# SteveMacenski/slam_toolbox

Measured on AMD Instinct MI355X. Metric: scan-matches/sec, higher is better.
Workload: dtype u8 gather / i32 sum / f64 penalty; 1 GPU; BASELINE config[1]: CorrelateScan 1081 beams 61x61x81 poses; parallelism=1 x independent match shards (no collective), streams_per_gpu=1

## Files before the change

### include/karto_hip.h

```cpp
#ifndef KARTO_HIP_H_
#define KARTO_HIP_H_

#include <stdint.h>

#ifdef __cplusplus
extern "C" {
#endif

#define KH_API __attribute__((visibility("default")))

enum {
  KH_OK = 0,
  KH_ERR_INVALID_ARG = 1,
  KH_ERR_NO_DEVICE = 2,
  KH_ERR_HIP = 3,
  KH_ERR_SEARCH = 4,
  KH_ERR_NOT_FOUND = 5,
  KH_ERR_SOLVER = 6,
  KH_ERR_IO = 7
};

KH_API const char * kh_last_error(void);
KH_API int kh_device_count(void);
KH_API const char * kh_version(void);
// ... 84 lines not shown
                                         double best_response, const double center[3], double angle_offset,
                                         double angle_resolution, double cov[9]);

typedef struct kh_grid_info {
  int32_t width, height, width_step, data_size;
  int32_t roi_x, roi_y, roi_w, roi_h;
  int32_t kernel_size;
  int32_t search_side;
  double offset_x, offset_y, scale;
} kh_grid_info;
KH_API int kh_matcher_grid_info(kh_matcher * m, int32_t slot, kh_grid_info * out);
KH_API int kh_matcher_read_grid(kh_matcher * m, int32_t slot, uint8_t * out );
KH_API int kh_matcher_read_kernel(kh_matcher * m, uint8_t * out );
KH_API int kh_matcher_read_lookup(kh_matcher * m, int32_t slot, int32_t * n_angles,
                                  int32_t * n_points, int32_t * out);
KH_API int kh_matcher_read_volume(kh_matcher * m, int32_t slot, int32_t * nx, int32_t * ny,
                                  int32_t * na, int32_t * out_sums, double * out_responses);
KH_API int kh_matcher_read_search_probabilities(kh_matcher * m, int32_t slot, int32_t * nx, int32_t * ny, double * out);
KH_API int kh_matcher_set_debug(kh_matcher * m, int32_t flags);
KH_API int kh_matcher_seq_stats(kh_matcher * m, int64_t out[8]);
KH_API void * kh_matcher_stream(kh_matcher * m);
KH_API int kh_matcher_profile(kh_matcher * m, int32_t enable, double * score_ms, int64_t * score_launches,
                              double * raster_ms, int64_t * raster_launches);

KH_API int kh_matcher_profile_side(kh_matcher * m, double * offsets_ms, double * ties_ms);

KH_API int kh_matcher_score_loads(kh_matcher * m, int64_t * wave_loads, int32_t reset);

typedef struct kh_spa kh_spa;

// ... 472 lines not shown
```

### slam_toolbox_amd/capi.py

```python
from __future__ import annotations

import ctypes as C
import os

import numpy as np

HERE = os.path.dirname(os.path.abspath(__file__))
LIB_PATH = os.environ.get("KH_LIBRARY") or os.path.join(HERE, "libkartohip.so")

KH_OK, KH_ERR_INVALID_ARG, KH_ERR_NO_DEVICE, KH_ERR_HIP, KH_ERR_SEARCH, KH_ERR_NOT_FOUND, KH_ERR_SOLVER, KH_ERR_IO = range(8)
KH_GRAPH_TEXT, KH_GRAPH_BINARY = 0, 1

dptr = np.ctypeslib.ndpointer(dtype=np.float64, flags="C_CONTIGUOUS")
iptr = np.ctypeslib.ndpointer(dtype=np.int32, flags="C_CONTIGUOUS")
bptr = np.ctypeslib.ndpointer(dtype=np.uint8, flags="C_CONTIGUOUS")


class KhScan(C.Structure):
    _fields_ = [("n", C.c_int32), ("ranges", C.POINTER(C.c_double)), ("points_xy", C.POINTER(C.c_double)),
                ("sensor_pose", C.c_double * 3), ("device_points_xy", C.c_void_p)]


class KhMatchParams(C.Structure):
    _fields_ = [("coarse_search_angle_offset", C.c_double), ("coarse_angle_resolution", C.c_double),
# ... 69 lines not shown
KH_SPA_MAX_COV_COLUMNS = 64


class KhMarginalizeSummary(C.Structure):
    _fields_ = [(k, C.c_int32) for k in ("n_marginalized", "n_plain", "n_rounds", "n_added", "n_fused", "max_degree")] + \
               [(k, C.c_double) for k in ("pack_ms", "kernel_ms", "apply_ms", "total_ms")]


KH_REMOVE_PLAIN, KH_REMOVE_MARGINALIZE = 0, 1


SYMBOLS = [
    "kh_last_error", "kh_device_count", "kh_version", "kh_scan_points", "kh_match_params_default",
    "kh_matcher_create", "kh_matcher_destroy", "kh_matcher_set_params", "kh_matcher_match",
    "kh_matcher_match_batch", "kh_matcher_add_scans", "kh_matcher_correlate", "kh_matcher_correlate_batch",
    "kh_matcher_grid_info", "kh_matcher_read_grid", "kh_matcher_read_kernel", "kh_matcher_read_lookup",
    "kh_matcher_positional_covariance", "kh_matcher_angular_covariance",
    "kh_matcher_read_volume", "kh_matcher_read_search_probabilities", "kh_matcher_set_debug", "kh_matcher_stream", "kh_matcher_profile", "kh_matcher_score_loads", "kh_matcher_seq_stats", "kh_matcher_profile_side",
    "kh_matcher_group_create", "kh_matcher_group_destroy", "kh_matcher_group_set_params", "kh_matcher_group_size", "kh_matcher_group_member",
    "kh_matcher_group_device", "kh_matcher_group_match_batch", "kh_loop_closure_batch",
    "kh_spa_options_default", "kh_spa_create", "kh_spa_set_debug", "kh_spa_destroy", "kh_spa_set_options", "kh_spa_reset",
    "kh_spa_clear", "kh_spa_add_node", "kh_spa_add_constraint", "kh_spa_remove_node",
    "kh_spa_remove_constraint", "kh_spa_modify_node", "kh_spa_get_node", "kh_spa_num_nodes",
    "kh_spa_num_constraints", "kh_spa_compute", "kh_spa_iteration_log", "kh_spa_get_corrections", "kh_link_info", "kh_spa_set_sharding",
    "kh_spa_save", "kh_spa_load", "kh_spa_add_constraint_information", "kh_spa_get_node_at", "kh_spa_get_constraint", "kh_spa_get_nodes",
    "kh_graph_create", "kh_graph_destroy", "kh_graph_set", "kh_graph_set_positions", "kh_graph_find_loop_candidates",
    "kh_graph_last_kernel_ms", "kh_graph_find_near_chains", "kh_graph_closest_scan_to_pose", "kh_weighted_mean",
    "kh_occupancy_compute_dimensions", "kh_occupancy_create", "kh_occupancy_destroy", "kh_occupancy_clear",
    "kh_occupancy_add_scans", "kh_occupancy_update", "kh_occupancy_read", "kh_occupancy_info",
    "kh_decay_params_default", "kh_lifelong_scores", "kh_lifelong_scores_resident",
    "kh_spa_set_comm", "kh_comm_unique_id", "kh_comm_create", "kh_comm_destroy", "kh_comm_rank", "kh_comm_world", "kh_comm_device",
# ... 187 lines not shown
        L.kh_matcher_group_member.argtypes = [vp, i32]
        L.kh_matcher_group_member.restype = vp
        L.kh_matcher_group_device.argtypes = [vp, i32]
        L.kh_matcher_group_match_batch.argtypes = [vp, i32, C.POINTER(KhScan), C.POINTER(KhScan), iptr, vp, i32, i32, dptr, dptr, dptr, iptr]
        L.kh_loop_closure_batch.argtypes = [vp, vp, i32, C.POINTER(KhScan), C.POINTER(KhScan), iptr, dbl, dbl, dbl, dbl, i32,
                                            dptr, dptr, dptr, iptr, dptr, dptr, dptr]
    L.kh_matcher_add_scans.argtypes = [vp, i32, C.POINTER(KhScan), C.POINTER(KhScan), i32]
    L.kh_matcher_correlate.argtypes = [vp, i32, C.POINTER(KhScan), dptr, dptr, dptr, dbl, dbl, i32, i32, dptr, dptr, C.POINTER(dbl)]
    L.kh_matcher_correlate_batch.argtypes = [vp, i32, C.POINTER(KhScan), dptr, dptr, dptr, dbl, dbl, i32, i32, dptr, dptr, dptr, iptr]
    L.kh_matcher_positional_covariance.argtypes = [vp, i32, dptr, dbl, dptr, dptr, dptr, dbl, dptr]
    L.kh_matcher_angular_covariance.argtypes = [vp, i32, C.POINTER(KhScan), dptr, dbl, dptr, dbl, dbl, dptr]
    L.kh_matcher_grid_info.argtypes = [vp, i32, C.POINTER(KhGridInfo)]
    L.kh_matcher_read_grid.argtypes = [vp, i32, bptr]
    L.kh_matcher_read_kernel.argtypes = [vp, bptr]
    L.kh_matcher_read_lookup.argtypes = [vp, i32, C.POINTER(i32), C.POINTER(i32), vp]
    L.kh_matcher_read_volume.argtypes = [vp, i32, C.POINTER(i32), C.POINTER(i32), C.POINTER(i32), vp, vp]
    if hasattr(L, "kh_matcher_read_search_probabilities"):
        L.kh_matcher_read_search_probabilities.argtypes = [vp, i32, C.POINTER(i32), C.POINTER(i32), vp]
    L.kh_matcher_set_debug.argtypes = [vp, i32]
    L.kh_matcher_stream.argtypes = [vp]
    L.kh_matcher_stream.restype = vp
    L.kh_matcher_profile.argtypes = [vp, i32, C.POINTER(dbl), C.POINTER(C.c_int64), C.POINTER(dbl), C.POINTER(C.c_int64)]
    L.kh_matcher_score_loads.argtypes = [vp, C.POINTER(C.c_int64), i32]
    L.kh_matcher_seq_stats.argtypes = [vp, C.POINTER(C.c_int64)]
    L.kh_matcher_profile_side.argtypes = [vp, C.POINTER(C.c_double), C.POINTER(C.c_double)]
    if hasattr(L, "kh_spa_create"):
        L.kh_spa_options_default.argtypes = [C.POINTER(KhSpaOptions)]
        L.kh_spa_create.argtypes = [i32, C.POINTER(vp)]
        L.kh_spa_destroy.argtypes = [vp]
        L.kh_spa_destroy.restype = None
# ... 219 lines not shown
```

### slam_toolbox_amd/csrc/kh_internal.hpp

```cpp
#pragma once
#include <cstddef>
#include <cstdint>

namespace kh
{

constexpr int32_t kInvalidScan = INT32_MAX;
constexpr int32_t kOccupied = 100;
constexpr int32_t kTieCap = 2048;
constexpr int32_t kGridPad = 512;
constexpr int32_t kTileBytes = 64;
constexpr int32_t kTileSpan = 61;
constexpr int32_t kClasses = 4;
constexpr int32_t kBlockShift = 5;
constexpr int32_t kCountsPerAngle = 8;
#ifndef KH_GROUP_ANGLES
#define KH_GROUP_ANGLES 2
#endif
#ifndef KH_LDS_PITCH
#define KH_LDS_PITCH 192
#endif
#ifndef KH_LDS_ROWS
#define KH_LDS_ROWS 196
#endif
// ... 94 lines not shown
  int32_t bm_w, bm_h, bshift;
  double * tile_best;
  int32_t * sums;
  double * resp;
  unsigned long long * out;
  int32_t out_words;
  const uint8_t * grid2;
  int32_t pitch2, copy_b;
  int32_t * fast2;
  int32_t * tcounts2;
  int32_t dec;
  int32_t pad_rows;
  int32_t pad;
  int32_t tile_px;
  unsigned long long * load_counter;
};

constexpr size_t kOutHeaderWords = 2 + kTieCap / 2;

struct ValidItem {int32_t job, scan;};
void launch_find_valid(const RasterJob * d_jobs, const ValidItem * d_items, int32_t n_items, int32_t max_n, void * stream);
void launch_active_set(const RasterJob * d_jobs, int32_t n_jobs, int32_t max_points, int32_t max_cap, void * stream);
void launch_raster(const RasterJob * d_jobs, int32_t n_jobs, int32_t max_points, int32_t max_tiles, const uint8_t * d_kernel, int32_t kernel_size,
  void * stream);
void launch_raster_clear(const RasterJob * d_jobs, int32_t n_jobs, void * stream);
void launch_repitch(const RasterJob * d_jobs, int32_t n_jobs, int32_t max_tiles, void * stream, bool any_copies);
void launch_repitch_full(const RasterJob * d_job, int32_t rows, void * stream);
void launch_offsets(const uint8_t * d_jobs, size_t stride, int32_t n_jobs, int32_t max_na, void * stream);
void launch_score(const uint8_t * d_jobs, size_t stride, int32_t n_jobs, int32_t max_tiles, int32_t max_na,
                  int32_t sx_variant, int32_t ry, void * stream);
__host__ __device__ inline int32_t lds_row_waves(int32_t ny) {return ny <= 16 ? 1 : ny <= 32 ? 2 : 4;}
inline int32_t score_tile_poses(int32_t sx) {return sx == 2 ? (kTileSpan + 1) / 2 : kTileSpan;}
void launch_offsets_lds(const uint8_t * d_jobs, size_t stride, int32_t n_jobs, int32_t max_na, void * stream);
void launch_score_lds(const uint8_t * d_jobs, size_t stride, int32_t n_jobs, int32_t max_na, int32_t sx_variant, bool full_rows, void * stream);
void launch_gather_small(const uint8_t * d_jobs, size_t stride, int32_t n_jobs, int32_t * d_out, int32_t small_stride, void * stream);
void launch_ties(const uint8_t * d_jobs, size_t stride, int32_t n_jobs, int32_t max_poses, int32_t tile_pairs, bool cells_in_score, void * stream);

}
```

### slam_toolbox_amd/csrc/matcher_device.hpp

```cpp
#pragma once
#include <hip/hip_runtime.h>
#include <atomic>
#include <cstdint>
#include "kh_internal.hpp"
#include "lds_attr.hpp"

namespace kh
{

__device__ __forceinline__ double d_round(double v) {return v >= 0.0 ? floor(v + 0.5) : ceil(v - 0.5);}
__device__ __forceinline__ int32_t d_to_int(double v)
{
  if (!(v > -2147483649.0 && v < 2147483648.0)) {return INT32_MIN;}
  return (int32_t)v;
}
__device__ __forceinline__ double2 job_point(const RasterJob & job, int p)
{
  if (job.uniform_n > 0) {
    const int k = p / job.uniform_n;
    return reinterpret_cast<const double2 *>(job.scan_ptr[k])[p - k * job.uniform_n];
  }
  int lo = 0, hi = job.n_scans;
  while (hi - lo > 1) {
    const int mid = (lo + hi) >> 1;
// ... 36 lines not shown
  const unsigned long long span = (1ull << nb) - 1ull;
  typedef __attribute__((address_space(1))) const uint32_t gword;
  gword * const words = (gword *)bmp + wi;
  constexpr int kRowsAtOnce = 9;
  unsigned long long any = 0;
  for (int by = by0; by <= by1; by += kRowsAtOnce) {
    uint32_t lo[kRowsAtOnce], hi[kRowsAtOnce];
#pragma unroll
    for (int k = 0; k < kRowsAtOnce; ++k) {
      gword * row = words + (size_t)min(by + k, by1) * bm_w;
      lo[k] = row[0]; hi[k] = row[1];
    }
#pragma unroll
    for (int k = 0; k < kRowsAtOnce; ++k) {any |= ((unsigned long long)hi[k] << 32) | lo[k];}
  }
  return ((any >> sh) & span) != 0;
}

template <bool kWaveSearch>
__device__ __forceinline__ void find_valid_scan(const double2 * pts, const int n, uint8_t * out, const double vx, const double vy,
  const int max_n, double2 * s_fv, uint8_t *& flags_lds, long long * dbg = nullptr)
{
#define KH_FV_STAMP(k) do {if (dbg && threadIdx.x == 0) {dbg[k] = (long long)wall_clock64();}} while (0)
  const int tid = threadIdx.x, lane = tid & 63, nthreads = blockDim.x;
  const int stride_i = max_n + 64;
  double2 * P = s_fv;
  int32_t * nxt0 = reinterpret_cast<int32_t *>(P + max_n);
  int32_t * nxa = nxt0 + stride_i;
  int32_t * nxb = nxa + stride_i;
  uint8_t * reach = reinterpret_cast<uint8_t *>(nxb + stride_i);
// ... 225 lines not shown
```

### slam_toolbox_amd/csrc/matcher_host.cpp

```cpp
#include "matcher_private.hpp"
#include "matcher_seq.hpp"

namespace kh
{
thread_local std::string g_last_error;
void set_error(const std::string & s) {g_last_error = s;}
}


namespace kh
{

static int32_t half_kernel_size(double smear, double resolution)
{
  return static_cast<int32_t>(round_half_away(2.0 * smear / resolution));
}


void host_parallel_for(size_t n, const std::function<void(size_t)> & fn) {HostPool::instance().run(n, fn);}
void host_parallel_for_wide(size_t n, const std::function<void(size_t)> & fn) {HostPool::wide().run(n, fn);}

void fill_raster_job(const kh_matcher * m, const Slot & s, const double * pose, int32_t n_points, size_t npad, RasterJob & j)
{
  std::memset(&j, 0, sizeof(j));
  j.grid = s.d_grid;
  j.view_x = pose[0]; j.view_y = pose[1];
  j.active = s.d_ractive; j.n_points = n_points;
  j.ws = m->ws; j.roi_x = m->roi_x; j.roi_y = m->roi_y; j.roi_w = m->roi_w; j.roi_h = m->roi_h;
  j.kernel_size = m->kernel_size; j.off_x = s.off_x; j.off_y = s.off_y; j.scale = m->scale;
  j.blockmap = s.d_blockmap; j.bm_w = m->bm_w; j.bm_h = m->bm_h; j.bshift = m->bshift;
  const size_t nt = static_cast<size_t>(m->rt_w) * m->rt_h;
  j.tiles_w = m->rt_w; j.tiles_h = m->rt_h; j.height = m->data_size / m->ws;
  j.tile_count = s.d_rtiles; j.tile_cursor = s.d_rtiles + nt; j.n_work = s.d_rtiles + 2 * nt;
  j.tile_start = s.d_rtiles + 2 * nt + 4; j.work = s.d_rtiles + 3 * nt + 4;
  j.cell_xy = s.d_rlists; j.list = s.d_rlists + 2 * npad; j.rank = s.d_rlists + 6 * npad;
  j.grid2 = s.d_grid2; j.copy_kind = s.copy_kind; j.prev_work = s.d_prev_work;
  j.pitch2 = s.copy_kind == 2 ? m->pitch_d : m->pitch2; j.copy_b = s.copy_kind == 2 ? m->copy_q : m->copy_b;
  j.n_foot = static_cast<int32_t>(m->footprint100.size()) - 1;
// ... 519 lines not shown
  job->grid_off_x = s.off_x; job->grid_off_y = s.off_y; job->scale = m->scale;
  job->bx = reinterpret_cast<const int32_t *>(db + L.bx);
  job->by = reinterpret_cast<const int32_t *>(db + L.by);
  job->dist_pen = L.dist_pen_bytes ? reinterpret_cast<const double *>(db + L.dist_pen) : c.geo->d_dist_pen;
  job->ang_pen = reinterpret_cast<const double *>(db + L.ang_pen);
  job->cos_sin = reinterpret_cast<const double *>(db + L.cos_sin);
  job->local = reinterpret_cast<const double *>(db + L.local);
  job->invalid = db + L.invalid;
  job->table = s.d_table; job->fast = s.d_fast; job->slow = s.d_slow; job->counts = s.d_counts;
  job->tcounts = s.d_tcounts; {
    const int32_t tiles = job->tiles_x * job->tiles_y;
    job->list_tiles = (tiles >= 4 && tiles <= c.lt_alloc) ? tiles : 1;
  }
  job->sums = s.d_sums; job->resp = s.d_resp; job->out = d_out; job->out_words = static_cast<int32_t>(out_words);
  job->blockmap = m->dense_score ? nullptr : s.d_blockmap; job->bm_w = m->bm_w; job->bm_h = m->bm_h; job->bshift = m->bshift;
  job->tile_best = s.d_tile_best;
  {
    const bool use2 = dec || (s.copy_kind == 1 && m->dual_copy && linear && (job->tiles_x == 1 || job->list_tiles > 1));
    const size_t lists = static_cast<size_t>(c.na) * kClasses * static_cast<size_t>(c.lt_alloc);
    job->grid2 = use2 ? s.d_grid2 : nullptr;
    job->pitch2 = dec ? m->pitch_d : m->pitch2; job->copy_b = dec ? m->copy_q : m->copy_b;
    job->fast2 = s.d_fast + lists * static_cast<size_t>(c.P);
    job->tcounts2 = s.d_tcounts + lists;
  }
  job->pad = std::max(0, m->pad_rows * m->ws - 512); job->pad_rows = m->pad_rows;
  job->load_counter = m->profiling ? m->d_load_counter : nullptr;
}

int finalize_job(kh_matcher * m, CorrReq & q, CorrHost & c, const ResultView & v)
{
// ... 171 lines not shown
    std::fprintf(stderr, "[kh corr] job 0: %d x %d x %d poses, sx %d, tiles %d x %d of %d x %d poses, lists per tile %d, copies %d (slot kind %d), "
      "dec %d, ws %d\n", j0->nx, j0->ny, j0->na, j0->sx, j0->tiles_x, j0->tiles_y, j0->tile_px, 4 * j0->ry, j0->list_tiles,
      j0->grid2 ? 1 : 0, m->slots[B.ctx[0].slot].copy_kind, j0->dec, m->ws);
  }
  int32_t max_tiles = 0, sx_variant = shapes[0].sx, ry = shapes[0].ry;
  const int32_t lds_sx = shapes[0].lds_sx;
  bool uniform_kernel = true, all_lds = true;
  for (size_t i = 0; i < n; ++i) {
    if (sx_variant != shapes[i].sx || ry != shapes[i].ry) {uniform_kernel = false;}
    all_lds = all_lds && shapes[i].lds_sx == lds_sx;
    max_tiles = std::max(max_tiles, shapes[i].tiles);
    all_lds = all_lds && shapes[i].lds != 0;
  }
  B.use_lds = all_lds && uniform_kernel;
  int32_t tile_pairs = 0;
  for (size_t i = 0; i < n; ++i) {
    CorrJob * job = reinterpret_cast<CorrJob *>(B.h_stage + stride * i);
    if (B.use_lds) {
      job->tiles_x = 1; job->tiles_y = 1; job->ry = 16; job->tile_px = kTileSpan;
      job->cells_in_score = 1;
    }
    tile_pairs = std::max(tile_pairs, job->na * job->tiles_x * job->tiles_y);
  }

  timing.lap(0, t_enter);
  const auto t_enqueue = std::chrono::steady_clock::now();
  hipStream_t cs = overlap ? B.side : m->stream;
  KH_HIP(hipMemcpyAsync(B.d_stage, B.h_stage, stride * n, hipMemcpyHostToDevice, cs));
  if (m->profiling) {KH_HIP(hipEventRecord(B.evs[0], cs));}
  if (B.use_lds) {
    launch_offsets_lds(B.d_stage, stride, static_cast<int32_t>(n), max_na, cs);
  } else {
    launch_offsets(B.d_stage, stride, static_cast<int32_t>(n), max_na, cs);
  }
  if (m->profiling) {KH_HIP(hipEventRecord(B.evs[1], cs));}
  if (m->profiling) {KH_HIP(hipEventRecord(B.ev[0], cs));}
  if (B.use_lds) {
    bool full_rows = true;
    for (size_t i = 0; i < n; ++i) {full_rows = full_rows && lds_row_waves(B.ctx[i].ny) == 4;}
    launch_score_lds(B.d_stage, stride, static_cast<int32_t>(n), max_na, lds_sx, full_rows, cs);
  } else if (uniform_kernel) {
    launch_score(B.d_stage, stride, static_cast<int32_t>(n), max_tiles, max_na, sx_variant, ry, cs);
  } else {
    for (size_t i = 0; i < n; ++i) {
      const CorrJob * job = reinterpret_cast<const CorrJob *>(B.h_stage + stride * i);
// ... 281 lines not shown
  }
  m->rt_w = (m->ws + kRasterTile - 1) / kRasterTile;
  m->rt_h = (m->data_size / m->ws + kRasterTile - 1) / kRasterTile;
  m->bshift = (m->kernel_size <= 25 && m->side <= 64 && max_batch >= 8) ? 3 : kBlockShift;
  m->bm_w = (((m->ws >> m->bshift) + 1) + 31) / 32 + 1;
  m->bm_h = (m->data_size / m->ws >> m->bshift) + 2;
  {
    const double table_bytes = 4.0 * static_cast<double>(m->roi_w) * m->roi_h * max_batch;
    m->table_raster = table_bytes <= 24e9 && m->rt_w * m->rt_h <= 16384;
  }
  m->slots.resize(max_batch);
  for (auto & s : m->slots) {
    if ((e = hipMalloc(reinterpret_cast<void **>(&s.d_grid_alloc), static_cast<size_t>(m->data_size) + 2 * m->grid_pad)) != hipSuccess) {return fail(e, "hipMalloc grid");}
    if ((e = hipMemset(s.d_grid_alloc, 0, static_cast<size_t>(m->data_size) + 2 * m->grid_pad)) != hipSuccess) {return fail(e, "hipMemset grid");}
    s.d_grid = s.d_grid_alloc + m->grid_pad;
    if ((e = hipMalloc(reinterpret_cast<void **>(&s.d_blockmap), static_cast<size_t>(m->bm_w) * m->bm_h * 4)) != hipSuccess) {return fail(e, "hipMalloc block map");}
    if ((e = hipMemset(s.d_blockmap, 0, static_cast<size_t>(m->bm_w) * m->bm_h * 4)) != hipSuccess) {return fail(e, "hipMemset block map");}
    if ((e = hipMalloc(reinterpret_cast<void **>(&s.d_rtiles), (4 * static_cast<size_t>(m->rt_w) * m->rt_h + 8) * sizeof(int32_t))) != hipSuccess) {return fail(e, "hipMalloc raster tiles");}
    const size_t prev_bytes = (static_cast<size_t>(m->rt_w) * m->rt_h + 4) * sizeof(int32_t);
    if ((e = hipMalloc(reinterpret_cast<void **>(&s.d_prev_work), prev_bytes)) != hipSuccess) {return fail(e, "hipMalloc tile list");}
    if ((e = hipMemset(s.d_prev_work, 0, prev_bytes)) != hipSuccess) {return fail(e, "hipMemset tile list");}
  }
  if ((e = hipHostMalloc(reinterpret_cast<void **>(&m->h_rjobs), sizeof(RasterJob) * max_batch, hipHostMallocDefault)) != hipSuccess) {return fail(e, "hipHostMalloc");}
  if ((e = hipMalloc(reinterpret_cast<void **>(&m->d_rjobs), sizeof(RasterJob) * max_batch)) != hipSuccess) {return fail(e, "hipMalloc");}
  *out = m;
  return KH_OK;
}

void kh_matcher_destroy(kh_matcher * m)
{
  if (!m) {return;}
  hipSetDevice(m->device);
// ... 271 lines not shown
  KH_HIP(hipMemcpy(out, m->d_kernel, m->kernel.size(), hipMemcpyDeviceToHost));
  return KH_OK;
}

int kh_matcher_read_lookup(kh_matcher * m, int32_t slot, int32_t * n_angles, int32_t * n_points, int32_t * out)
{
  if (!m || slot < 0 || slot >= m->max_batch || !n_angles || !n_points) {return KH_ERR_INVALID_ARG;}
  Slot & s = m->slots[slot];
  if (!s.has_last) {return KH_ERR_NOT_FOUND;}
  *n_angles = s.last.na; *n_points = s.last.P;
  if (out) {
    KH_HIP(hipSetDevice(m->device));
    KH_HIP(hipStreamSynchronize(m->stream));
    KH_HIP(hipMemcpy(out, s.d_table, sizeof(int32_t) * s.last.na * s.last.P, hipMemcpyDeviceToHost));
  }
  return KH_OK;
}

int kh_matcher_read_volume(kh_matcher * m, int32_t slot, int32_t * nx, int32_t * ny, int32_t * na,
  int32_t * out_sums, double * out_responses)
{
  if (!m || slot < 0 || slot >= m->max_batch || !nx || !ny || !na) {return KH_ERR_INVALID_ARG;}
  Slot & s = m->slots[slot];
  if (!s.has_last) {return KH_ERR_NOT_FOUND;}
  if (s.volume_stale) {set_error("the last search re-scored an off-lattice best pose: its volume was not kept"); return KH_ERR_NOT_FOUND;}
  const auto & c = s.last;
  *nx = c.nx; *ny = c.ny; *na = c.na;
  if (!out_sums && !out_responses) {return KH_OK;}
  KH_HIP(hipSetDevice(m->device));
  KH_HIP(hipStreamSynchronize(m->stream));
// ... 110 lines not shown
```

### slam_toolbox_amd/csrc/matcher_kernels.hip

```cpp
#include <hip/hip_runtime.h>
#include <algorithm>
#include <atomic>
#include <cstdint>
#include <cstdlib>
#include "kh_internal.hpp"
#include "matcher_device.hpp"

namespace kh
{

constexpr int kCodeWords = 128;
__global__ __launch_bounds__(64) void k_find_valid_lane(const RasterJob * jobs, const ValidItem * items, int n_items)
{
  __shared__ uint32_t s_codes[kCodeWords][64];
  const int t = blockIdx.x * blockDim.x + threadIdx.x;
  if (t >= n_items) {return;}
  const int lane = threadIdx.x;
  const RasterJob & job = jobs[items[t].job];
  const int k = items[t].scan;
  const int n = job.scan_prefix[k + 1] - job.scan_prefix[k];
  const double2 * pts = reinterpret_cast<const double2 *>(job.scan_ptr[k]);
  uint8_t * out = job.active + job.scan_prefix[k];
  const bool in_lds = n <= 16 * kCodeWords;
  const double vx = job.view_x, vy = job.view_y;
// ... 1231 lines not shown
__device__ __forceinline__ int wave_prefix(int v)
{
  constexpr int ident = kMin ? INT32_MAX : INT32_MIN;
  auto op = [](int x, int y) {return kMin ? (y < x ? y : x) : (y > x ? y : x);};
  v = op(v, __builtin_amdgcn_update_dpp(ident, v, 0x111, 0xf, 0xf, false));
  v = op(v, __builtin_amdgcn_update_dpp(ident, v, 0x112, 0xf, 0xf, false));
  v = op(v, __builtin_amdgcn_update_dpp(ident, v, 0x114, 0xf, 0xf, false));
  v = op(v, __builtin_amdgcn_update_dpp(ident, v, 0x118, 0xf, 0xf, false));
  v = op(v, __builtin_amdgcn_update_dpp(ident, v, 0x142, 0xa, 0xf, false));
  v = op(v, __builtin_amdgcn_update_dpp(ident, v, 0x143, 0xc, 0xf, false));
  return v;
}
__device__ __forceinline__ int wave_prefix_min(int v, int) {return wave_prefix<true>(v);}
__device__ __forceinline__ int wave_prefix_max(int v, int) {return wave_prefix<false>(v);}

__global__ __launch_bounds__(256) void k_offsets_lds(const uint8_t * jobs, size_t stride)
{
  const CorrJob & job = *reinterpret_cast<const CorrJob *>(jobs + (size_t)blockIdx.y * stride);
  const int group = blockIdx.x;
  const int a0 = group * kGroupAngles;
  if (a0 >= job.na) {return;}
  {
    const int groups = (job.na + kGroupAngles - 1) / kGroupAngles;
    const int per = (job.out_words + groups - 1) / groups;
    const int hi = min(job.out_words, (group + 1) * per);
    for (int i = group * per + threadIdx.x; i < hi; i += blockDim.x) {job.out[i] = 0ull;}
  }
  const int P = job.n_points;
  __shared__ int32_t s_slow[kGroupAngles];
  if (threadIdx.x < kGroupAngles) {s_slow[threadIdx.x] = 0;}
// ... 13 lines not shown
  double cosine[kGroupAngles], sine[kGroupAngles];
#pragma unroll
  for (int q = 0; q < kGroupAngles; ++q) {
    cosine[q] = a0 + q < na ? job.cos_sin[2 * (a0 + q)] : 1.0;
    sine[q] = a0 + q < na ? job.cos_sin[2 * (a0 + q) + 1] : 0.0;
  }
  int32_t * const table = job.table;
  int32_t * const slow = job.slow;
  int32_t * const rel_out = job.rel;
  const int rounds = (P + 255) / 256;
  const int desc_cap = lds_desc_capacity(P);
  ChunkDesc * out = reinterpret_cast<ChunkDesc *>(job.chunks) + ((size_t)group * kLdsRanges + wave) * desc_cap;
  int n_out = 0;
  long long windows_total = 0;
  constexpr int kMaxRounds = 8;
  double plx[kMaxRounds], ply[kMaxRounds];
  bool pinv[kMaxRounds];
  {
    typedef __attribute__((address_space(1))) const uint8_t gflag;
    typedef __attribute__((address_space(1))) const double gdouble;
    gflag * const ginvalid = (gflag *)job.invalid;
    gdouble * const glocal = (gdouble *)job.local;
    uint8_t fl[kMaxRounds];
#pragma unroll
    for (int t = 0; t < kMaxRounds; ++t) {
      const int ic = min((int)threadIdx.x + 256 * t, P - 1);
      fl[t] = ginvalid[ic]; plx[t] = glocal[2 * ic]; ply[t] = glocal[2 * ic + 1];
    }
#pragma unroll
    for (int t = 0; t < kMaxRounds; ++t) {
      const int i = threadIdx.x + 256 * t;
      const bool in = t < rounds && i < P;
      pinv[t] = in ? fl[t] != 0 : true;
      plx[t] = in ? plx[t] : 0.0;
      ply[t] = in ? ply[t] : 0.0;
    }
  }
#pragma unroll
  for (int t = 0; t < kMaxRounds; ++t) {
    if (t >= rounds) {break;}
    const int i = threadIdx.x + 256 * t;
    const bool inr = i < P;
    int gx[kGroupAngles], gy[kGroupAngles];
#pragma unroll
    for (int q = 0; q < kGroupAngles; ++q) {
      gx[q] = 0; gy[q] = kNotFast;
      if (!inr || a0 + q >= na) {continue;}
      int32_t idx;
      if (pinv[t]) {
        idx = kInvalidScan;
      } else {
        const double lx = plx[t], ly = ply[t];
        const double ox = cosine[q] * lx - sine[q] * ly;
        const double oy = sine[q] * lx + cosine[q] * ly;
        const double gxd = ((ox + off_x) - off_x) * scale;
        const double gyd = ((oy + off_y) - off_y) * scale;
        const int32_t gxi = d_to_int(d_round(gxd));
        const int32_t gyi = d_to_int(d_round(gyd));
        idx = (int32_t)((uint32_t)gxi + (uint32_t)gyi * (uint32_t)ws);
        if (idx != kInvalidScan) {
          const bool off_grid = (int64_t)idx + bmax < 0 || (int64_t)idx + bmin >= data_size;
          const bool inside = (int64_t)idx + bmin >= -pad && (int64_t)idx + bmax < data_size + pad;
          const bool exact = (int64_t)gxi + (int64_t)gyi * ws == (int64_t)idx && gxi > -(1 << 20) && gxi < (1 << 20);
          if (!off_grid) {
            if (inside && exact) {
              gx[q] = gxi; gy[q] = gyi;
              if (bmp) {
                const int32_t start = (int32_t)((int64_t)idx + bmin);
                int32_t wy0 = (int32_t)((float)start * inv_ws);
                int32_t wx0 = start - wy0 * ws;
                while (wx0 < 0) {wx0 += ws; --wy0;}
                while (wx0 >= ws) {wx0 -= ws; ++wy0;}
                if (wx0 + xs <= ws && !window_has_blocks(bmp, bm_w, bm_h, wx0, wy0, wx0 + xs - 1, wy0 + ys - 1, bshift)) {
                  gy[q] = kNotFast;
                }
              }
            } else {
              (slow + (size_t)(a0 + q) * P)[atomicAdd(&s_slow[q], 1)] = idx;
            }
          }
        }
      }
      table[(size_t)(a0 + q) * P + i] = idx;
    }
    const int run_lo = i - lane;
    const int n_run = min(64, P - run_lo);
    int begin = 0;
    while (begin < n_run) {
      const bool live_lane = lane >= begin && lane < n_run;
      int n = 0, x0 = 0, y0 = 0, rows = 0;
      bool any_chunk = false;
      for (;;) {
        int xmin = INT32_MAX, xmax = INT32_MIN, ymin = INT32_MAX, ymax = INT32_MIN;
#pragma unroll
        for (int q = 0; q < kGroupAngles; ++q) {
          if (live_lane && gy[q] != kNotFast) {
            xmin = min(xmin, gx[q]); xmax = max(xmax, gx[q]); ymin = min(ymin, gy[q]); ymax = max(ymax, gy[q]);
          }
        }
// ... 50 lines not shown
            if (cls == c) {my_rank = offset + __popcll(mask & ((1ull << lane) - 1ull));}
            offset += cnt;
            packed |= cnt << (8 * c);
          }
          d.cnt[q] = packed;
          windows += offset;
          if (mine) {rel_out[(size_t)a * P + run_lo + begin + my_rank] = rel & ~3;}
        }
        d.windows = windows;
        windows_total += windows;
        if (lane == 0) {out[n_out] = d;}
        ++n_out;
      }
      begin += n;
    }
  }
  if (lane == 0) {
    job.chunk_counts[(size_t)group * kLdsRanges + wave] = n_out;
    if (job.load_counter && windows_total) {atomicAdd(job.load_counter, (unsigned long long)(windows_total * 4 * row_waves));}
  }
  __syncthreads();
  if (threadIdx.x < kGroupAngles && a0 + (int)threadIdx.x < job.na) {
    job.counts[kCountsPerAngle * (a0 + threadIdx.x) + kClasses] = s_slow[threadIdx.x];
  }
}

void launch_offsets_lds(const uint8_t * d_jobs, size_t stride, int32_t n_jobs, int32_t max_na, void * stream)
{
  if (n_jobs <= 0 || max_na <= 0) {return;}
  const int groups = (max_na + kGroupAngles - 1) / kGroupAngles;
// ... 352 lines not shown
```

### slam_toolbox_amd/csrc/matcher_private.hpp

```cpp
#pragma once
#include <hip/hip_runtime.h>

#include <algorithm>
#include <atomic>
#include <chrono>
#include <cmath>
#include <condition_variable>
#include <cstdint>
#include <cstdio>
#include <cstdlib>
#include <cstring>
#include <functional>
#include <memory>
#include <mutex>
#include <string>
#include <thread>
#include <unordered_map>
#include <unordered_set>
#include <vector>

#include "../../include/karto_hip.h"
#include "kh_internal.hpp"
#include "host_pool.hpp"
#include "covariance_walk.hpp"
// ... 86 lines not shown
  unsigned long long * d_out = nullptr; size_t cap_dout = 0;
  int32_t * h_sums = nullptr; size_t cap_hsums = 0;
  int32_t * d_small = nullptr; size_t cap_dsmall = 0; size_t small_stride = 0;
  hipEvent_t ev[2] = {nullptr, nullptr};
  hipEvent_t evs[4] = {nullptr, nullptr, nullptr, nullptr};
  hipEvent_t done = nullptr;
  hipEvent_t kdone = nullptr;
  hipStream_t side = nullptr;
};

struct Slot
{
  uint8_t * d_grid = nullptr;
  uint8_t * d_grid_alloc = nullptr;
  uint32_t * d_blockmap = nullptr;
  uint8_t * d_grid2 = nullptr;
  uint8_t * d_grid2_alloc = nullptr;
  int32_t copy_kind = 0;
  int32_t * d_prev_work = nullptr;
  double off_x = 0.0, off_y = 0.0;
  int32_t * d_table = nullptr, * d_fast = nullptr, * d_slow = nullptr, * d_counts = nullptr;
  int32_t * d_tcounts = nullptr; size_t cap_tcounts = 0, cap_fast = 0;
  size_t cap_table = 0, cap_counts = 0;
  int32_t * d_chunks = nullptr, * d_chunk_counts = nullptr; size_t cap_chunks = 0, cap_chunk_counts = 0;
  int32_t * d_sums = nullptr; double * d_resp = nullptr; size_t cap_volume = 0, cap_resp = 0;
  uint8_t * d_ractive = nullptr; size_t cap_ractive = 0;
  uint32_t * d_hkeys = nullptr; int32_t * d_hvals = nullptr; uint8_t * d_hstate = nullptr; int32_t * d_hnbr = nullptr;
  size_t cap_hkeys = 0, cap_hvals = 0, cap_hstate = 0, cap_hnbr = 0;
  double * d_tile_best = nullptr; size_t cap_tile_best = 0;
  int32_t * d_rtiles = nullptr;
// ... 138 lines not shown
CorrReq fine_search(const kh_matcher * m, int32_t slot, const kh_scan * query, const double * center, bool penalize);
struct TablePlan {bool ok = false; int reason = 0; size_t bin_lds = 0; bool bm_global = false;};
TablePlan plan_table_raster(const kh_matcher * m, int64_t most_points, int32_t most_readings, int32_t n_scans);
struct QueryHook
{
  std::function<void()> fn;
  void run() {if (fn) {std::function<void()> f; f.swap(fn); f();}}
};
QueryHook & pending_query_hook();
int seq_match(kh_matcher * m, const kh_scan * query, const kh_scan * base, int32_t n_base, bool penalize, bool refine,
  double mean[3], double cov[9], double * response, int * status, bool * coarse_done, bool * fine_done);
void seq_destroy(kh_matcher * m);
constexpr int kSeqStatWords = 8;
enum {kSeqStatCalls = 0, kSeqStatFineOnDevice = 1, kSeqStatFineFallback = 2, kSeqStatFineMismatch = 3, kSeqStatCoarseFallback = 4, kSeqStatFusedScore = 5};
const int64_t * seq_stats(const kh_matcher * m);
void fill_raster_job(const kh_matcher * m, const Slot & s, const double * pose, int32_t n_points, size_t npad, RasterJob & j);
int ensure_seq_tables(kh_matcher * m, Slot & s, int32_t n_points, RasterJob & j);

}
```

### slam_toolbox_amd/scan_matcher.py

```python
from __future__ import annotations

import ctypes as C
from dataclasses import dataclass

import numpy as np

from . import capi


@dataclass
class MapperParams:
    coarse_search_angle_offset: float = 20 * 0.01745329251994329577
    coarse_angle_resolution: float = 2 * 0.01745329251994329577
    fine_search_angle_offset: float = 0.2 * 0.01745329251994329577
    use_response_expansion: bool = False
    distance_variance_penalty: float = 0.3
    minimum_distance_penalty: float = 0.5
    angle_variance_penalty: float = 20 * 0.01745329251994329577
    minimum_angle_penalty: float = 0.9

    def c(self) -> capi.KhMatchParams:
        p = capi.KhMatchParams()
        p.coarse_search_angle_offset = self.coarse_search_angle_offset
        p.coarse_angle_resolution = self.coarse_angle_resolution
# ... 194 lines not shown
        capi.check(capi.lib().kh_matcher_read_grid(self._h, slot, out), "kh_matcher_read_grid")
        return out

    def kernel(self):
        k = self.grid_info()["kernel_size"]
        out = np.zeros(k * k, dtype=np.uint8)
        capi.check(capi.lib().kh_matcher_read_kernel(self._h, out), "kh_matcher_read_kernel")
        return out.reshape(k, k)

    def lookup_table(self, slot=0):
        na, npnt = C.c_int32(), C.c_int32()
        capi.check(capi.lib().kh_matcher_read_lookup(self._h, slot, C.byref(na), C.byref(npnt), None), "read_lookup")
        out = np.zeros((na.value, npnt.value), dtype=np.int32)
        capi.check(capi.lib().kh_matcher_read_lookup(self._h, slot, C.byref(na), C.byref(npnt),
                                                     out.ctypes.data_as(C.c_void_p)), "read_lookup")
        return out

    def set_debug(self, keep_response_volume: bool, lds_score: bool = False, dense_score: bool = False,
                  force_chunks: bool = False, no_dual_copy: bool = False, windowed_score: bool = False,
                  no_fused_match: bool = False):
        capi.check(capi.lib().kh_matcher_set_debug(self._h, int(bool(keep_response_volume)) | (2 if lds_score else 0) |
                                                   (4 if dense_score else 0) | (8 if force_chunks else 0) |
                                                   (16 if no_dual_copy else 0) | (64 if windowed_score else 0) |
                                                   (128 if no_fused_match else 0)),
                   "kh_matcher_set_debug")

    def volume(self, slot=0, responses=True):
        nx, ny, na = C.c_int32(), C.c_int32(), C.c_int32()
        capi.check(capi.lib().kh_matcher_read_volume(self._h, slot, C.byref(nx), C.byref(ny), C.byref(na), None, None),
                   "read_volume")
# ... 122 lines not shown
```

Before: 120,700 scan-matches/s.

## Add hierarchical block-map levels for constant-probe window emptiness tests

Builds power-of-two row-OR levels of the occupancy block map on the device, lazily, whenever the grid changes. The offsets kernel can then test window emptiness with two 64-bit probes instead of scanning every block row. Probes for several rounds are batched so their loads can be issued together. The cost is an extra level-build kernel per grid update, more block-map memory, and more register pressure in the offsets kernel. A debug reader for the block-map levels is also added.

```diff
diff --git a/include/karto_hip.h b/include/karto_hip.h
--- a/include/karto_hip.h
+++ b/include/karto_hip.h
@@ -122,6 +122,7 @@
 KH_API int kh_matcher_read_kernel(kh_matcher * m, uint8_t * out );
 KH_API int kh_matcher_read_lookup(kh_matcher * m, int32_t slot, int32_t * n_angles,
                                   int32_t * n_points, int32_t * out);
+KH_API int kh_matcher_read_blockmap(kh_matcher * m, int32_t slot, int32_t level, int32_t * bm_w, int32_t * bm_h, uint32_t * out);
 KH_API int kh_matcher_read_volume(kh_matcher * m, int32_t slot, int32_t * nx, int32_t * ny,
                                   int32_t * na, int32_t * out_sums, double * out_responses);
 KH_API int kh_matcher_read_search_probabilities(kh_matcher * m, int32_t slot, int32_t * nx, int32_t * ny, double * out);
diff --git a/slam_toolbox_amd/capi.py b/slam_toolbox_amd/capi.py
--- a/slam_toolbox_amd/capi.py
+++ b/slam_toolbox_amd/capi.py
@@ -107,7 +107,7 @@
     "kh_last_error", "kh_device_count", "kh_version", "kh_scan_points", "kh_match_params_default",
     "kh_matcher_create", "kh_matcher_destroy", "kh_matcher_set_params", "kh_matcher_match",
     "kh_matcher_match_batch", "kh_matcher_add_scans", "kh_matcher_correlate", "kh_matcher_correlate_batch",
-    "kh_matcher_grid_info", "kh_matcher_read_grid", "kh_matcher_read_kernel", "kh_matcher_read_lookup",
+    "kh_matcher_grid_info", "kh_matcher_read_grid", "kh_matcher_read_kernel", "kh_matcher_read_lookup", "kh_matcher_read_blockmap",
     "kh_matcher_positional_covariance", "kh_matcher_angular_covariance",
     "kh_matcher_read_volume", "kh_matcher_read_search_probabilities", "kh_matcher_set_debug", "kh_matcher_stream", "kh_matcher_profile", "kh_matcher_score_loads", "kh_matcher_seq_stats", "kh_matcher_profile_side",
     "kh_matcher_group_create", "kh_matcher_group_destroy", "kh_matcher_group_set_params", "kh_matcher_group_size", "kh_matcher_group_member",
@@ -325,6 +325,8 @@
     L.kh_matcher_read_grid.argtypes = [vp, i32, bptr]
     L.kh_matcher_read_kernel.argtypes = [vp, bptr]
     L.kh_matcher_read_lookup.argtypes = [vp, i32, C.POINTER(i32), C.POINTER(i32), vp]
+    if hasattr(L, "kh_matcher_read_blockmap"):
+        L.kh_matcher_read_blockmap.argtypes = [vp, i32, i32, C.POINTER(i32), C.POINTER(i32), vp]
     L.kh_matcher_read_volume.argtypes = [vp, i32, C.POINTER(i32), C.POINTER(i32), C.POINTER(i32), vp, vp]
     if hasattr(L, "kh_matcher_read_search_probabilities"):
         L.kh_matcher_read_search_probabilities.argtypes = [vp, i32, C.POINTER(i32), C.POINTER(i32), vp]
diff --git a/slam_toolbox_amd/csrc/kh_internal.hpp b/slam_toolbox_amd/csrc/kh_internal.hpp
--- a/slam_toolbox_amd/csrc/kh_internal.hpp
+++ b/slam_toolbox_amd/csrc/kh_internal.hpp
@@ -132,7 +132,11 @@
   int32_t pad;
   int32_t tile_px;
   unsigned long long * load_counter;
+  const uint32_t * bm_levels;
+  int32_t level_mask;
+  int32_t build_levels;
 };
+constexpr int32_t kBlockLevels = 3;
 
 constexpr size_t kOutHeaderWords = 2 + kTieCap / 2;
 
@@ -150,6 +154,7 @@
 __host__ __device__ inline int32_t lds_row_waves(int32_t ny) {return ny <= 16 ? 1 : ny <= 32 ? 2 : 4;}
 inline int32_t score_tile_poses(int32_t sx) {return sx == 2 ? (kTileSpan + 1) / 2 : kTileSpan;}
 void launch_offsets_lds(const uint8_t * d_jobs, size_t stride, int32_t n_jobs, int32_t max_na, void * stream);
+void launch_blockmap_levels(const uint8_t * d_jobs, size_t stride, int32_t n_jobs, uint32_t * single, int32_t single_build, int32_t bm_w, int32_t bm_h, void * stream);
 void launch_score_lds(const uint8_t * d_jobs, size_t stride, int32_t n_jobs, int32_t max_na, int32_t sx_variant, bool full_rows, void * stream);
 void launch_gather_small(const uint8_t * d_jobs, size_t stride, int32_t n_jobs, int32_t * d_out, int32_t small_stride, void * stream);
 void launch_ties(const uint8_t * d_jobs, size_t stride, int32_t n_jobs, int32_t max_poses, int32_t tile_pairs, bool cells_in_score, void * stream);
diff --git a/slam_toolbox_amd/csrc/matcher_device.hpp b/slam_toolbox_amd/csrc/matcher_device.hpp
--- a/slam_toolbox_amd/csrc/matcher_device.hpp
+++ b/slam_toolbox_amd/csrc/matcher_device.hpp
@@ -74,6 +74,35 @@
 #pragma unroll
     for (int k = 0; k < kRowsAtOnce; ++k) {any |= ((unsigned long long)hi[k] << 32) | lo[k];}
   }
+  return ((any >> sh) & span) != 0;
+}
+
+constexpr int kProbeEmpty = 0;
+constexpr int kProbeKeep = 1;
+constexpr int kProbeLevels = 2;
+constexpr int kProbeRows = 3;
+__device__ __forceinline__ int block_probe_plan(int bm_w, int bm_h, int x_lo, int y_lo, int x_hi, int y_hi, int bshift, int level_mask, int & off_a, int & key)
+{
+  const int bx0 = x_lo >> bshift, bx1 = x_hi >> bshift;
+  const int by0 = max(y_lo, 0) >> bshift, by1 = min(y_hi >> bshift, bm_h - 1);
+  const int wi = bx0 >> 5, sh = bx0 & 31, nb = bx1 - bx0 + 1;
+  if (nb > 32) {return kProbeKeep;}
+  if (by1 < by0) {return kProbeEmpty;}
+  const int n = by1 - by0 + 1;
+  if (n > 16) {return kProbeRows;}
+  const int k = min(31 - __clz(n), kBlockLevels);
+  if (((level_mask >> k) & 1) == 0) {return kProbeRows;}
+  const int plane = k * bm_h;
+  off_a = (plane + by0) * bm_w + wi;
+  key = sh | (nb << 8) | ((n - (1 << k)) << 16);
+  return kProbeLevels;
+}
+__device__ __forceinline__ int block_probe_second(int off_a, int key, int bm_w) {return key >= 0 ? off_a + (key >> 16) * bm_w : off_a;}
+__device__ __forceinline__ bool block_probe_hit(int key, uint32_t a_lo, uint32_t a_hi, uint32_t b_lo, uint32_t b_hi)
+{
+  const int sh = key & 31, nb = (key >> 8) & 63;
+  const unsigned long long span = (1ull << nb) - 1ull;
+  const unsigned long long any = ((unsigned long long)(a_hi | b_hi) << 32) | (a_lo | b_lo);
   return ((any >> sh) & span) != 0;
 }
 
diff --git a/slam_toolbox_amd/csrc/matcher_host.cpp b/slam_toolbox_amd/csrc/matcher_host.cpp
--- a/slam_toolbox_amd/csrc/matcher_host.cpp
+++ b/slam_toolbox_amd/csrc/matcher_host.cpp
@@ -20,8 +20,9 @@
 void host_parallel_for(size_t n, const std::function<void(size_t)> & fn) {HostPool::instance().run(n, fn);}
 void host_parallel_for_wide(size_t n, const std::function<void(size_t)> & fn) {HostPool::wide().run(n, fn);}
 
-void fill_raster_job(const kh_matcher * m, const Slot & s, const double * pose, int32_t n_points, size_t npad, RasterJob & j)
-{
+void fill_raster_job(const kh_matcher * m, Slot & s, const double * pose, int32_t n_points, size_t npad, RasterJob & j)
+{
+  ++s.bm_writes;
   std::memset(&j, 0, sizeof(j));
   j.grid = s.d_grid;
   j.view_x = pose[0]; j.view_y = pose[1];
@@ -571,6 +572,7 @@
   }
   job->sums = s.d_sums; job->resp = s.d_resp; job->out = d_out; job->out_words = static_cast<int32_t>(out_words);
   job->blockmap = m->dense_score ? nullptr : s.d_blockmap; job->bm_w = m->bm_w; job->bm_h = m->bm_h; job->bshift = m->bshift;
+  job->bm_levels = nullptr; job->level_mask = 0; job->build_levels = 0;
   job->tile_best = s.d_tile_best;
   {
     const bool use2 = dec || (s.copy_kind == 1 && m->dual_copy && linear && (job->tiles_x == 1 || job->list_tiles > 1));
@@ -772,8 +774,26 @@
   }
   B.use_lds = all_lds && uniform_kernel;
   int32_t tile_pairs = 0;
+  bool stale_levels = false;
   for (size_t i = 0; i < n; ++i) {
     CorrJob * job = reinterpret_cast<CorrJob *>(B.h_stage + stride * i);
+    if (B.use_lds && job->blockmap) {
+      Slot & s = m->slots[B.ctx[i].slot];
+      job->bm_levels = s.d_blockmap + static_cast<size_t>(m->bm_w) * m->bm_h;
+      const int32_t ys = (job->ny - 1) * job->sy_cells + 1, side = 1 << m->bshift;
+      const int32_t n_lo = ((ys - 1) >> m->bshift) + 1, n_hi = ((ys - 2 + side) >> m->bshift) + 1;
+      int32_t want = 1;
+      for (int32_t rows : {n_lo, n_hi}) {
+        int32_t k = 0;
+        while (k < kBlockLevels && (2 << k) <= rows) {++k;}
+        if (rows <= 16) {want |= 1 << k;}
+      }
+      job->level_mask = 1;
+      for (int32_t k = 1; k <= kBlockLevels; ++k) {
+        if (((want >> k) & 1) && s.levels_at[k] != s.bm_writes) {job->build_levels |= 1 << k; s.levels_at[k] = s.bm_writes; stale_levels = true;}
+        if (s.levels_at[k] == s.bm_writes) {job->level_mask |= 1 << k;}
+      }
+    }
     if (B.use_lds) {
       job->tiles_x = 1; job->tiles_y = 1; job->ry = 16; job->tile_px = kTileSpan;
       job->cells_in_score = 1;
@@ -787,6 +807,7 @@
   KH_HIP(hipMemcpyAsync(B.d_stage, B.h_stage, stride * n, hipMemcpyHostToDevice, cs));
   if (m->profiling) {KH_HIP(hipEventRecord(B.evs[0], cs));}
   if (B.use_lds) {
+    if (stale_levels) {launch_blockmap_levels(B.d_stage, stride, static_cast<int32_t>(n), nullptr, 0, m->bm_w, m->bm_h, cs);}
     launch_offsets_lds(B.d_stage, stride, static_cast<int32_t>(n), max_na, cs);
   } else {
     launch_offsets(B.d_stage, stride, static_cast<int32_t>(n), max_na, cs);
@@ -1098,8 +1119,8 @@
     if ((e = hipMalloc(reinterpret_cast<void **>(&s.d_grid_alloc), static_cast<size_t>(m->data_size) + 2 * m->grid_pad)) != hipSuccess) {return fail(e, "hipMalloc grid");}
     if ((e = hipMemset(s.d_grid_alloc, 0, static_cast<size_t>(m->data_size) + 2 * m->grid_pad)) != hipSuccess) {return fail(e, "hipMemset grid");}
     s.d_grid = s.d_grid_alloc + m->grid_pad;
-    if ((e = hipMalloc(reinterpret_cast<void **>(&s.d_blockmap), static_cast<size_t>(m->bm_w) * m->bm_h * 4)) != hipSuccess) {return fail(e, "hipMalloc block map");}
-    if ((e = hipMemset(s.d_blockmap, 0, static_cast<size_t>(m->bm_w) * m->bm_h * 4)) != hipSuccess) {return fail(e, "hipMemset block map");}
+    if ((e = hipMalloc(reinterpret_cast<void **>(&s.d_blockmap), static_cast<size_t>(m->bm_w) * m->bm_h * 4 * (1 + kBlockLevels))) != hipSuccess) {return fail(e, "hipMalloc block map");}
+    if ((e = hipMemset(s.d_blockmap, 0, static_cast<size_t>(m->bm_w) * m->bm_h * 4 * (1 + kBlockLevels))) != hipSuccess) {return fail(e, "hipMemset block map");}
     if ((e = hipMalloc(reinterpret_cast<void **>(&s.d_rtiles), (4 * static_cast<size_t>(m->rt_w) * m->rt_h + 8) * sizeof(int32_t))) != hipSuccess) {return fail(e, "hipMalloc raster tiles");}
     const size_t prev_bytes = (static_cast<size_t>(m->rt_w) * m->rt_h + 4) * sizeof(int32_t);
     if ((e = hipMalloc(reinterpret_cast<void **>(&s.d_prev_work), prev_bytes)) != hipSuccess) {return fail(e, "hipMalloc tile list");}
@@ -1401,6 +1422,27 @@
     KH_HIP(hipStreamSynchronize(m->stream));
     KH_HIP(hipMemcpy(out, s.d_table, sizeof(int32_t) * s.last.na * s.last.P, hipMemcpyDeviceToHost));
   }
+  return KH_OK;
+}
+
+int kh_matcher_read_blockmap(kh_matcher * m, int32_t slot, int32_t level, int32_t * bm_w, int32_t * bm_h, uint32_t * out)
+{
+  if (!m || slot < 0 || slot >= m->max_batch || !bm_w || !bm_h || level < 0 || level > kBlockLevels) {return KH_ERR_INVALID_ARG;}
+  *bm_w = m->bm_w; *bm_h = m->bm_h;
+  if (!out) {return KH_OK;}
+  Slot & s = m->slots[slot];
+  const size_t plane = static_cast<size_t>(m->bm_w) * m->bm_h;
+  KH_HIP(hipSetDevice(m->device));
+  KH_HIP(hipStreamSynchronize(m->stream));
+  if (level > 0 && s.levels_at[level] != s.bm_writes) {
+    int32_t build = 0;
+    for (int32_t k = 1; k <= kBlockLevels; ++k) {build |= s.levels_at[k] != s.bm_writes ? 1 << k : 0;}
+    launch_blockmap_levels(nullptr, 0, 1, s.d_blockmap, build, m->bm_w, m->bm_h, m->stream);
+    KH_HIP(hipGetLastError());
+    KH_HIP(hipStreamSynchronize(m->stream));
+    for (int32_t k = 1; k <= kBlockLevels; ++k) {s.levels_at[k] = s.bm_writes;}
+  }
+  KH_HIP(hipMemcpy(out, s.d_blockmap + plane * level, plane * 4, hipMemcpyDeviceToHost));
   return KH_OK;
 }
 
diff --git a/slam_toolbox_amd/csrc/matcher_kernels.hip b/slam_toolbox_amd/csrc/matcher_kernels.hip
--- a/slam_toolbox_amd/csrc/matcher_kernels.hip
+++ b/slam_toolbox_amd/csrc/matcher_kernels.hip
@@ -1269,6 +1269,48 @@
 __device__ __forceinline__ int wave_prefix_min(int v, int) {return wave_prefix<true>(v);}
 __device__ __forceinline__ int wave_prefix_max(int v, int) {return wave_prefix<false>(v);}
 
+constexpr int kLevelSeg = 8;
+__global__ __launch_bounds__(64) void k_blockmap_levels(const uint8_t * jobs, size_t stride, uint32_t * single, int single_build, int bm_w, int bm_h)
+{
+  uint32_t * bm = single;
+  int build = single_build;
+  if (jobs) {
+    const CorrJob & job = *reinterpret_cast<const CorrJob *>(jobs + (size_t)blockIdx.y * stride);
+    if (!job.build_levels || !job.bm_levels) {return;}
+    build = job.build_levels;
+    bm = const_cast<uint32_t *>(job.bm_levels) - (size_t)bm_w * bm_h;
+  }
+  const int item = blockIdx.x * 64 + threadIdx.x;
+  const int segs = (bm_h + kLevelSeg - 1) / kLevelSeg;
+  if (item >= segs * bm_w) {return;}
+  const int w = item % bm_w, by_s = (item / bm_w) * kLevelSeg;
+  uint32_t r[kLevelSeg + 7];
+#pragma unroll
+  for (int j = 0; j < kLevelSeg + 7; ++j) {r[j] = bm[(size_t)min(by_s + j, bm_h - 1) * bm_w + w];}
+#pragma unroll
+  for (int i = 0; i < kLevelSeg; ++i) {
+    const int by = by_s + i;
+    if (by >= bm_h) {break;}
+    const uint32_t l1 = r[i] | r[i + 1];
+    const uint32_t l2 = l1 | r[i + 2] | r[i + 3];
+    const uint32_t l3 = l2 | r[i + 4] | r[i + 5] | r[i + 6] | r[i + 7];
+    if (build & 2) {bm[((size_t)1 * bm_h + by) * bm_w + w] = l1;}
+    if (build & 4) {bm[((size_t)2 * bm_h + by) * bm_w + w] = l2;}
+    if (build & 8) {bm[((size_t)3 * bm_h + by) * bm_w + w] = l3;}
+  }
+}
+
+void launch_blockmap_levels(const uint8_t * d_jobs, size_t stride, int32_t n_jobs, uint32_t * single, int32_t single_build, int32_t bm_w, int32_t bm_h, void * stream)
+{
+  if (n_jobs <= 0 || bm_w <= 0 || bm_h <= 0) {return;}
+  const int items = ((bm_h + kLevelSeg - 1) / kLevelSeg) * bm_w;
+  hipLaunchKernelGGL(k_blockmap_levels, dim3((items + 63) / 64, n_jobs), dim3(64), 0, (hipStream_t)stream, d_jobs, stride, single, single_build, bm_w, bm_h);
+}
+
+#ifndef KH_PROBE_ROUNDS
+#define KH_PROBE_ROUNDS 4
+#endif
+
 __global__ __launch_bounds__(256) void k_offsets_lds(const uint8_t * jobs, size_t stride)
 {
   const CorrJob & job = *reinterpret_cast<const CorrJob *>(jobs + (size_t)blockIdx.y * stride);
@@ -1312,8 +1354,9 @@
   int n_out = 0;
   long long windows_total = 0;
   constexpr int kMaxRounds = 8;
+  constexpr int kProbeRounds = KH_PROBE_ROUNDS;
   double plx[kMaxRounds], ply[kMaxRounds];
-  bool pinv[kMaxRounds];
+  uint32_t pinv = 0;
   {
     typedef __attribute__((address_space(1))) const uint8_t gflag;
     typedef __attribute__((address_space(1))) const double gdouble;
@@ -1329,23 +1372,34 @@
     for (int t = 0; t < kMaxRounds; ++t) {
       const int i = threadIdx.x + 256 * t;
       const bool in = t < rounds && i < P;
-      pinv[t] = in ? fl[t] != 0 : true;
+      pinv |= (in ? fl[t] != 0 : true) ? 1u << t : 0u;
       plx[t] = in ? plx[t] : 0.0;
       ply[t] = in ? ply[t] : 0.0;
     }
   }
-#pragma unroll
-  for (int t = 0; t < kMaxRounds; ++t) {
-    if (t >= rounds) {break;}
-    const int i = threadIdx.x + 256 * t;
-    const bool inr = i < P;
-    int gx[kGroupAngles], gy[kGroupAngles];
+  typedef __attribute__((address_space(1))) const uint32_t gword;
+  gword * const gbm = (gword *)bmp;
+  const bool have_levels = job.bm_levels != nullptr;
+  const int level_mask = job.level_mask;
+#pragma unroll
+  for (int t0 = 0; t0 < kMaxRounds; t0 += kProbeRounds) {
+  if (t0 >= rounds) {break;}
+  int gxs[kProbeRounds][kGroupAngles], gys[kProbeRounds][kGroupAngles];
+  int probe_a[kProbeRounds][kGroupAngles], probe_key[kProbeRounds][kGroupAngles];
+#pragma unroll
+  for (int u = 0; u < kProbeRounds; ++u) {
+    const int t = min(t0 + u, kMaxRounds - 1);
+    int (&gx)[kGroupAngles] = gxs[u];
+    int (&gy)[kGroupAngles] = gys[u];
+    const int i = threadIdx.x + 256 * (t0 + u);
+    const bool inr = t0 + u < rounds && i < P;
 #pragma unroll
     for (int q = 0; q < kGroupAngles; ++q) {
       gx[q] = 0; gy[q] = kNotFast;
+      probe_a[u][q] = 0; probe_key[u][q] = -1;
       if (!inr || a0 + q >= na) {continue;}
       int32_t idx;
-      if (pinv[t]) {
+      if (pinv & (1u << t)) {
         idx = kInvalidScan;
       } else {
         const double lx = plx[t], ly = ply[t];
@@ -1369,8 +1423,14 @@
                 int32_t wx0 = start - wy0 * ws;
                 while (wx0 < 0) {wx0 += ws; --wy0;}
                 while (wx0 >= ws) {wx0 -= ws; ++wy0;}
-                if (wx0 + xs <= ws && !window_has_blocks(bmp, bm_w, bm_h, wx0, wy0, wx0 + xs - 1, wy0 + ys - 1, bshift)) {
-                  gy[q] = kNotFast;
+                if (wx0 + xs <= ws) {
+                  const int need = have_levels ?
+                    block_probe_plan(bm_w, bm_h, wx0, wy0, wx0 + xs - 1, wy0 + ys - 1, bshift, level_mask, probe_a[u][q], probe_key[u][q]) : kProbeRows;
+                  if (need == kProbeEmpty) {
+                    gy[q] = kNotFast;
+                  } else if (need == kProbeRows) {
+                    if (!window_has_blocks(bmp, bm_w, bm_h, wx0, wy0, wx0 + xs - 1, wy0 + ys - 1, bshift)) {gy[q] = kNotFast;}
+                  }
                 }
               }
             } else {
@@ -1381,6 +1441,34 @@
       }
       table[(size_t)(a0 + q) * P + i] = idx;
     }
+  }
+  if (have_levels) {
+    uint32_t pa_lo[kProbeRounds][kGroupAngles], pa_hi[kProbeRounds][kGroupAngles], pb_lo[kProbeRounds][kGroupAngles], pb_hi[kProbeRounds][kGroupAngles];
+#pragma unroll
+    for (int u = 0; u < kProbeRounds; ++u) {
+#pragma unroll
+      for (int q = 0; q < kGroupAngles; ++q) {
+        pa_lo[u][q] = gbm[probe_a[u][q]]; pa_hi[u][q] = gbm[probe_a[u][q] + 1];
+        const int probe_b = block_probe_second(probe_a[u][q], probe_key[u][q], bm_w);
+        pb_lo[u][q] = gbm[probe_b]; pb_hi[u][q] = gbm[probe_b + 1];
+      }
+    }
+#pragma unroll
+    for (int u = 0; u < kProbeRounds; ++u) {
+#pragma unroll
+      for (int q = 0; q < kGroupAngles; ++q) {
+        const bool hit = block_probe_hit(probe_key[u][q], pa_lo[u][q], pa_hi[u][q], pb_lo[u][q], pb_hi[u][q]);
+        gys[u][q] = (probe_key[u][q] >= 0 && !hit) ? kNotFast : gys[u][q];
+      }
+    }
+  }
+#pragma unroll
+  for (int u = 0; u < kProbeRounds; ++u) {
+    const int t = t0 + u;
+    if (t >= rounds) {break;}
+    int (&gx)[kGroupAngles] = gxs[u];
+    int (&gy)[kGroupAngles] = gys[u];
+    const int i = threadIdx.x + 256 * t;
     const int run_lo = i - lane;
     const int n_run = min(64, P - run_lo);
     int begin = 0;
@@ -1461,6 +1549,7 @@
       }
       begin += n;
     }
+  }
   }
   if (lane == 0) {
     job.chunk_counts[(size_t)group * kLdsRanges + wave] = n_out;
diff --git a/slam_toolbox_amd/csrc/matcher_private.hpp b/slam_toolbox_amd/csrc/matcher_private.hpp
--- a/slam_toolbox_amd/csrc/matcher_private.hpp
+++ b/slam_toolbox_amd/csrc/matcher_private.hpp
@@ -124,6 +124,8 @@
   uint8_t * d_grid = nullptr;
   uint8_t * d_grid_alloc = nullptr;
   uint32_t * d_blockmap = nullptr;
+  uint64_t bm_writes = 1;
+  uint64_t levels_at[1 + kBlockLevels] = {0, 0, 0, 0};
   uint8_t * d_grid2 = nullptr;
   uint8_t * d_grid2_alloc = nullptr;
   int32_t copy_kind = 0;
@@ -292,7 +294,7 @@
 constexpr int kSeqStatWords = 8;
 enum {kSeqStatCalls = 0, kSeqStatFineOnDevice = 1, kSeqStatFineFallback = 2, kSeqStatFineMismatch = 3, kSeqStatCoarseFallback = 4, kSeqStatFusedScore = 5};
 const int64_t * seq_stats(const kh_matcher * m);
-void fill_raster_job(const kh_matcher * m, const Slot & s, const double * pose, int32_t n_points, size_t npad, RasterJob & j);
+void fill_raster_job(const kh_matcher * m, Slot & s, const double * pose, int32_t n_points, size_t npad, RasterJob & j);
 int ensure_seq_tables(kh_matcher * m, Slot & s, int32_t n_points, RasterJob & j);
 
 }
diff --git a/slam_toolbox_amd/scan_matcher.py b/slam_toolbox_amd/scan_matcher.py
--- a/slam_toolbox_amd/scan_matcher.py
+++ b/slam_toolbox_amd/scan_matcher.py
@@ -232,6 +232,14 @@
         out = np.zeros((na.value, npnt.value), dtype=np.int32)
         capi.check(capi.lib().kh_matcher_read_lookup(self._h, slot, C.byref(na), C.byref(npnt),
                                                      out.ctypes.data_as(C.c_void_p)), "read_lookup")
+        return out
+
+    def blockmap(self, slot=0, level=0):
+        w, h = C.c_int32(), C.c_int32()
+        capi.check(capi.lib().kh_matcher_read_blockmap(self._h, slot, level, C.byref(w), C.byref(h), None), "read_blockmap")
+        out = np.zeros((h.value, w.value), dtype=np.uint32)
+        capi.check(capi.lib().kh_matcher_read_blockmap(self._h, slot, level, C.byref(w), C.byref(h),
+                                                       out.ctypes.data_as(C.c_void_p)), "read_blockmap")
         return out
 
     def set_debug(self, keep_response_volume: bool, lds_score: bool = False, dense_score: bool = False,
```

Measured after the change: 121,300 scan-matches/s (median of 2 runs). About the same (+0.5%).
